# jtdingx/quadrupedal_loco

Measured on AMD Instinct MI355X. Metric: MPC QP solves/sec (Go1 SRBD N=10, 12 forces); p99 solve us, higher is better.
Workload: dtype f32

## Files before the change

### quadrupedal_loco_amd/csrc/qloco_srbd_lit.hip

```cpp
#include <math.h>
#include <stddef.h>

#include <type_traits>

#include "qloco_srbd_core.hpp"
#include "qloco_srbd_model.hpp"
#include "qloco_srbd_place.hpp"

namespace qloco {

constexpr int kLitWpe = 4;
constexpr int kLit2Wpe = 2;

template <int W>
struct LitLds {
  static constexpr int NS = W == 1 ? kLitN : kLitN2;
  static constexpr int NT = NS;
  float Bb[6][12];
  float Te[6][6];
  float q2[16], r2[12], x0[16];
  float ctf[4 * NT];
  float pad0[W == 1 ? 0 : 24];
  f4v bc[W][W][16];
  float av[W][2][64];
  float wv[W][64];
  float zh[W][2][64];
  float dr[W][2][64];
  float qvl[W][2][64];
  f4v arz[W][2][64];
  union alignas(16) {
    struct {
      f2v beps[12][12];
      float dcol[12 * NT];
      float err[12 * NT];
      float Wc[12 * NT];
    };
    struct {
      float w0i[W][3][2][64];
      f2v gtab[NT][NT][3];
    };
  };
  f2v k0k2[NT][NT];
  struct {
    float rho, cs, cinv, qn0, qn1, alpha, oma, sigma, dtm;
    float zlo;
    float sxy[2][2];
    int iter, status, rho_updates, ctm, interval;
  } sc[W];
  float piv[W == 1 ? 0 : 2];
  float red[W == 1 ? 0 : 2][16];
};
static_assert(sizeof(LitLds<1>) <= 10240, "literal kernel: four workgroups per SIMD need <= 160 KB / 16 of LDS");
static_assert(sizeof(LitLds<2>) <= 40960, "two-wave literal kernel: four workgroups per CU need <= 40 KB");
static_assert(offsetof(LitLds<1>, dcol) % 16 == 0 && offsetof(LitLds<2>, dcol) % 16 == 0,
              "dcol is read as f4v (ds_read_b128 needs 16-byte alignment)");
static_assert(offsetof(LitLds<1>, Bb) % 16 == 0 && offsetof(LitLds<1>, bc) % 16 == 0 && offsetof(LitLds<1>, arz) % 16 == 0 &&
                  offsetof(LitLds<2>, Bb) % 16 == 0 && offsetof(LitLds<2>, bc) % 16 == 0 && offsetof(LitLds<2>, arz) % 16 == 0,
              "Bb rows, bc and arz are read as f4v");
static_assert((offsetof(LitLds<1>, w0i) - offsetof(LitLds<1>, bc)) % 256 == 0 &&
                  (offsetof(LitLds<2>, w0i) - offsetof(LitLds<2>, bc)) % 256 == 0 && offsetof(LitLds<1>, Bb) == 0,
              "the ADMM loop's two-address reads reach its per-lane arrays from one lane register");

__device__ __forceinline__ void lsync() {
  __builtin_amdgcn_fence(__ATOMIC_RELEASE, "wavefront");
  __builtin_amdgcn_wave_barrier();
  __builtin_amdgcn_fence(__ATOMIC_ACQUIRE, "wavefront");
}
template <int W>
__device__ __forceinline__ void bsync() {
  if constexpr (W == 1)
    lsync();
  else
    __syncthreads();
}

template <int W, int K>
__device__ __forceinline__ void bcombine_max(LitLds<W> &S, float (&v)[K], int wv) {
  if constexpr (W == 2) {
    static_assert(K <= 16, "red holds 16 partials per wave");
    if (__builtin_amdgcn_mbcnt_hi(~0u, __builtin_amdgcn_mbcnt_lo(~0u, 0u)) == 0) {
#pragma unroll
      for (int k = 0; k < K; ++k) S.red[wv][k] = v[k];
    }
    bsync<W>();
#pragma unroll
    for (int k = 0; k < K; ++k) v[k] = fmaxf(S.red[0][k], S.red[1][k]);
    bsync<W>();
  }
}
template <int W>
__device__ __forceinline__ float bsum(LitLds<W> &S, float v, int wv) {
  if constexpr (W == 2) {
    if (__builtin_amdgcn_mbcnt_hi(~0u, __builtin_amdgcn_mbcnt_lo(~0u, 0u)) == 0) S.red[wv][0] = v;
    bsync<W>();
    v = S.red[0][0] + S.red[1][0];
    bsync<W>();
  }
  return v;
}
template <int W>
__device__ __forceinline__ float bmax1(LitLds<W> &S, float v, int wv) {
  float t[1] = {v};
  bcombine_max<W, 1>(S, t, wv);
  return t[0];
}

struct Triple {
  float v0, v1, v2;
};
__device__ __forceinline__ Triple triple(float v, int comp) {
  const float n1 = lane_next(v), n2 = lane_next(n1);
  const float p1 = lane_prev(v), p2 = lane_prev(p1);
  Triple t;
  t.v0 = comp == 0 ? v : (comp == 1 ? p1 : p2);
  t.v1 = comp == 0 ? n1 : (comp == 1 ? v : p1);
  t.v2 = comp == 0 ? n2 : (comp == 1 ? n1 : v);
  return t;
}

struct Shift5 {
  float cm2, cm1, c0, cp1, cp2;
};
__device__ __forceinline__ Shift5 shift5(float a0, float a1, float a2, int comp) {
  Shift5 c;
  c.c0 = comp == 0 ? a0 : (comp == 1 ? a1 : a2);
  c.cm1 = comp == 1 ? a0 : (comp == 2 ? a1 : 0.0f);
  c.cm2 = comp == 2 ? a0 : 0.0f;
  c.cp1 = comp == 0 ? a1 : (comp == 1 ? a2 : 0.0f);
  c.cp2 = comp == 0 ? a2 : 0.0f;
  return c;
}
__device__ __forceinline__ float tdot(float v, const Shift5 &c) {
  float a, t, u;
  asm("s_nop 1\n\t"
      "v_mov_b32_dpp %1, %3 wave_shr:1 row_mask:0xf bank_mask:0xf bound_ctrl:0\n\t"
      "v_mov_b32_dpp %2, %3 wave_shl:1 row_mask:0xf bank_mask:0xf bound_ctrl:0\n\t"
      "v_mul_f32 %0, %3, %4\n\t"
      "v_fmac_f32_dpp %0, %3, %5 wave_shr:1 row_mask:0xf bank_mask:0xf bound_ctrl:0\n\t"
      "v_fmac_f32_dpp %0, %3, %7 wave_shl:1 row_mask:0xf bank_mask:0xf bound_ctrl:0\n\t"
      "v_fmac_f32_dpp %0, %1, %6 wave_shr:1 row_mask:0xf bank_mask:0xf bound_ctrl:0\n\t"
      "v_fmac_f32_dpp %0, %2, %8 wave_shl:1 row_mask:0xf bank_mask:0xf bound_ctrl:0"
      : "=&v"(a), "=&v"(t), "=&v"(u)
      : "v"(v), "v"(c.c0), "v"(c.cm1), "v"(c.cm2), "v"(c.cp1), "v"(c.cp2));
  return a;
}

__device__ __forceinline__ void tdot2(float v0, const Shift5 &c, float v1, const Shift5 &d, float &a0, float &a1) {
  float t0, t1, u0, u1;
  asm("s_nop 1\n\t"
      "v_mov_b32_dpp %2, %6 wave_shr:1 row_mask:0xf bank_mask:0xf bound_ctrl:0\n\t"
      "v_mov_b32_dpp %3, %7 wave_shr:1 row_mask:0xf bank_mask:0xf bound_ctrl:0\n\t"
      "v_mov_b32_dpp %4, %6 wave_shl:1 row_mask:0xf bank_mask:0xf bound_ctrl:0\n\t"
      "v_mov_b32_dpp %5, %7 wave_shl:1 row_mask:0xf bank_mask:0xf bound_ctrl:0\n\t"
      "v_mul_f32 %0, %6, %8\n\t"
      "v_mul_f32 %1, %7, %13\n\t"
      "v_fmac_f32_dpp %0, %6, %9 wave_shr:1 row_mask:0xf bank_mask:0xf bound_ctrl:0\n\t"
      "v_fmac_f32_dpp %1, %7, %14 wave_shr:1 row_mask:0xf bank_mask:0xf bound_ctrl:0\n\t"
      "v_fmac_f32_dpp %0, %6, %11 wave_shl:1 row_mask:0xf bank_mask:0xf bound_ctrl:0\n\t"
      "v_fmac_f32_dpp %1, %7, %16 wave_shl:1 row_mask:0xf bank_mask:0xf bound_ctrl:0\n\t"
      "v_fmac_f32_dpp %0, %2, %10 wave_shr:1 row_mask:0xf bank_mask:0xf bound_ctrl:0\n\t"
      "v_fmac_f32_dpp %1, %3, %15 wave_shr:1 row_mask:0xf bank_mask:0xf bound_ctrl:0\n\t"
      "v_fmac_f32_dpp %0, %4, %12 wave_shl:1 row_mask:0xf bank_mask:0xf bound_ctrl:0\n\t"
      "v_fmac_f32_dpp %1, %5, %17 wave_shl:1 row_mask:0xf bank_mask:0xf bound_ctrl:0"
      : "=&v"(a0), "=&v"(a1), "=&v"(t0), "=&v"(t1), "=&v"(u0), "=&v"(u1)
      : "v"(v0), "v"(v1), "v"(c.c0), "v"(c.cm1), "v"(c.cm2), "v"(c.cp1), "v"(c.cp2),
        "v"(d.c0), "v"(d.cm1), "v"(d.cm2), "v"(d.cp1), "v"(d.cp2));
}

__device__ __forceinline__ void lit_invert(LitLds<1> &S, int lane, int ncol, Row<1> &K) {
  int nc = __builtin_amdgcn_readfirstlane(ncol);
  {
    const float v = K.k[0];
    const float p = __builtin_bit_cast(float, __builtin_amdgcn_readlane(__builtin_bit_cast(int, v), 0));
    reinterpret_cast<float *>(&S.bc[0][0][0])[lane] = lane == 0 ? p + 1.0f : v;
  }
  ColLoop<0, 60>::run([&](auto kc) {
    constexpr int k = decltype(kc)::value;
    asm volatile("" : "+s"(nc));
    if (k >= nc) return;
    const bool is_k = __builtin_amdgcn_inverse_ballot_w64(1ull << k);
    lsync();
    const f4v r0 = S.bc[0][0][lane & 15];
    const float v = K.k[k];
    const float p = __builtin_bit_cast(float, __builtin_amdgcn_readlane(__builtin_bit_cast(int, v), k));
    const float pinv = __builtin_amdgcn_rcpf(p);
    const float ng = is_k ? pinv - 1.0f : -v * pinv;
    if constexpr (k + 1 < 60) {
      const bool is_k1 = __builtin_amdgcn_inverse_ballot_w64(1ull << (k + 1));
      const bool upto_k = __builtin_amdgcn_inverse_ballot_w64((2ull << k) - 1ull);
      const float la = fmaf(dpp_col<k + 1>(r0), ng, K.k[k + 1]);
      const float p1 = __builtin_bit_cast(float, __builtin_amdgcn_readlane(__builtin_bit_cast(int, la), k + 1));
      reinterpret_cast<float *>(&S.bc[0][0][0])[lane] = is_k1 ? p1 + 1.0f : (upto_k ? -la : la);
    }
    QL_DPP_GJ60_P1(K.k, 0, r0, ng);
    if (p > kGjExactPivot) K.k[k] = is_k ? pinv : ng;
  });
  lsync();
}

template <int HF, int KL>
__device__ __forceinline__ void lit2_pivot(LitLds<2> &S, int wv, int nc, Row<2> &K) {
  const int tt = fresh_lane();
  if constexpr (KL >= 1) {
    if (KL == nc) {
      constexpr int k1 = 60 * HF + KL - 1;
      const float v = K.k[k1];
      const bool own1 = wv == HF && tt == KL - 1;
      const bool before = HF == 0 && wv == 1;
      reinterpret_cast<float *>(&S.bc[k1 & 1][wv][0])[tt] = own1 ? v + 1.0f : (before ? -v : v);
      if (own1) S.piv[k1 & 1] = v;
    }
  }
  if constexpr (KL < 60) {
    constexpr int k = 60 * HF + KL;
    constexpr int pb = k & 1;
    if (KL >= nc) return;
    bsync<2>();
    const f4v r0 = S.bc[pb][0][tt & 15];
    const f4v r1 = S.bc[pb][1][tt & 15];
    const float p = S.piv[pb];
    const float v = K.k[k];
    const float pinv = __builtin_amdgcn_rcpf(p);
    const bool own = wv == HF && tt == KL;
    const float ng = own ? pinv - 1.0f : -v * pinv;
    if constexpr (KL >= 1) {
      const float la = fmaf(dpp_col<KL - 1>(HF ? r1 : r0), ng, K.k[k - 1]);
      const bool own1 = wv == HF && tt == KL - 1;
      const bool before = HF ? (wv == 1 && tt >= KL) : (wv == 1 || tt >= KL);
      reinterpret_cast<float *>(&S.bc[pb ^ 1][wv][0])[tt] = own1 ? la + 1.0f : (before ? -la : la);
      if (own1) S.piv[pb ^ 1] = la;
    }
    QL_DPP_GJ60(K.k, 0, r0, ng);
    QL_DPP_GJ60(K.k, 60, r1, ng);
    if (p > kGjExactPivot) K.k[k] = own ? pinv : ng;
  }
}

__device__ __forceinline__ void lit_invert2(LitLds<2> &S, int wv, int nc0, int nc1, Row<2> &K) {
  nc0 = __builtin_amdgcn_readfirstlane(nc0);
  nc1 = __builtin_amdgcn_readfirstlane(nc1);
  ColLoop<0, 61>::run([&](auto kc) {
    asm volatile("" : "+s"(nc1));
    lit2_pivot<1, 60 - decltype(kc)::value>(S, wv, nc1, K);
  });
  ColLoop<0, 61>::run([&](auto kc) {
    asm volatile("" : "+s"(nc0));
    lit2_pivot<0, 60 - decltype(kc)::value>(S, wv, nc0, K);
  });
  bsync<2>();
}

#define QL_LIT_LANE_INDICES(LX)                                                                    \
  const int LX = fresh_lane();                                                                     \
  const int jr = LX < 60 ? LX / 6 : kLitN - 1, sr = LX < 60 ? LX - 6 * (LX / 6) : 0;               \
  const int jc = W == 1 ? jr : 10 * wv + jr;                                                       \
  const bool wvalid = LX < nw;                                                                     \
  const int step[2] = {LX < 60 && LX < nvl ? so + LX / 12 : so, LX < 60 && 60 + LX < nvl ? so + (60 + LX) / 12 : so}; \
  const int stepl[2] = {step[0] - so, step[1] - so};                                               \
  const int leg[2] = {LX < 60 && LX < nvl ? (LX % 12) / 3 : 0, LX < 60 && 60 + LX < nvl ? ((60 + LX) % 12) / 3 : 0}; \
  const int comp = LX % 3;                                                                         \
  const bool xy = comp < 2;                                                                        \
  const bool valid[2] = {LX < 60 && LX < nvl, LX < 60 && 60 + LX < nvl};                           \
  (void)jr; (void)sr; (void)jc; (void)wvalid; (void)stepl; (void)step; (void)leg; (void)comp; (void)xy; (void)valid

template <int W, bool WS, bool MR>
__device__ __forceinline__ void srbd_lit_one(const SrbdArgs &a, LitLds<W> &S, const int64_t b) {
  constexpr int NS = LitLds<W>::NS, NT = LitLds<W>::NT;
  const int lane = W == 1 ? (int)threadIdx.x : (int)(threadIdx.x & 63);
  const int tid = threadIdx.x;
  const int wv = W == 1 ? 0 : __builtin_amdgcn_readfirstlane((int)(threadIdx.x >> 6));
  const int N = a.N;
  const float Nf = (float)N;
  const float dt = a.dt;
  SrbdBodyAt<MR> body{a};
  auto load_body = [&] {
    if constexpr (MR) {
      int64_t bb = b;
      asm volatile("" : "+s"(bb));
      body.row = srbd_body(a, bb);
    }
  };
  if constexpr (MR) {
    body.row = srbd_body(a, b);
    if (srbd_body_bad(body.row)) {
      srbd_refuse<64 * W>(a, b, W == 1 ? fresh_lane() : opaque_tid(), QLOCO_ERR_ARG);
      return;
    }
  }
  const float dtm = dt / body.mass(), dt2m = dt * dt / body.mass();
  const int H = W == 1 ? N : (N + 1) / 2;
  const int so = W == 1 ? 0 : wv * H;
  const int Nw = W == 1 ? N : (wv ? N - H : H);
  const int nvar = 12 * N, nvl = 12 * Nw, nw = 6 * Nw;

  if (tid < 13) S.x0[tid] = a.x0[b * 13 + tid];
  if (tid == 0) {
#pragma unroll
    for (int k = 0; k < 13; ++k) S.q2[k] = a.q2[k];
#pragma unroll
    for (int k = 0; k < 12; ++k) S.r2[k] = a.r2[k];
  }
  {
    const int nct = a.contacts_per_step ? 4 * N : 4;
    if (tid < 4 * N) S.ctf[tid] = a.contacts[b * nct + (a.contacts_per_step ? tid : (tid & 3))] ? 1.0f : 0.0f;
  }
  for (int idx = tid; idx < NT * NT; idx += 64 * W) {
    const int sr = idx / NT, sc = idx - NT * sr;
    float K0 = 0.0f, K2 = 0.0f;
    if constexpr (W == 1) {
      if (sr < N && sc < N) k0k2((float)sr, (float)sc, Nf, K0, K2);
    } else {
      const int gr = sr % 10 < (sr >= 10 ? N - H : H) ? (sr >= 10 ? H : 0) + sr % 10 : -1;
      const int gc = sc % 10 < (sc >= 10 ? N - H : H) ? (sc >= 10 ? H : 0) + sc % 10 : -1;
      if (gr >= 0 && gc >= 0) k0k2((float)gr, (float)gc, Nf, K0, K2);
    }
    S.k0k2[sr][sc] = (f2v){K0, K2};
  }
  if constexpr (W == 2) {
    for (int idx = tid; idx < 12 * NT; idx += 64 * W) S.dcol[idx] = 0.0f;
  }
  bsync<W>();

  const float yaw = S.x0[2];
  float sy, cy;
  sincosf(yaw, &sy, &cy);
  const float R00 = cy, R01 = sy, R10 = -sy, R11 = cy;
  if constexpr (W == 1) {
    if (a.lit_tables && tid == 0) {
      const float sq = a.lit_sq;
      S.sc[0].sxy[0][0] = sq * cy;
      S.sc[0].sxy[0][1] = -(sq * sy);
      S.sc[0].sxy[1][0] = sq * sy;
      S.sc[0].sxy[1][1] = sq * cy;
    }
  }
  float Ii[3][3];
  srbd_inertia_inv(cy, sy, body.inertia(), Ii);
  const int comp = lane % 3;
  const bool xy = comp < 2;
  bool valid[2];
  int step[2], leg[2], cst[2];
  f4v lo[2], hi[2];
#pragma unroll
  for (int h = 0; h < 2; ++h) {
    const int v = 60 * h + lane;
    valid[h] = lane < 60 && v < nvl;
    step[h] = valid[h] ? so + v / 12 : 0;
    cst[h] = W == 1 ? step[h] : (valid[h] ? 10 * wv + v / 12 : 0);
    leg[h] = valid[h] ? (v % 12) / 3 : 0;
    float ba[3];
    srbd_bd_column(Ii, srbd_foot(a.feet, b, N, 0, step[h], leg[h]), comp, dt, R00, R01, R10, R11,
                   step[h], valid[h], ba, lo[h], hi[h]);
    if (h == 0 && tid < 12) {
      S.Bb[0][lane] = ba[0];
      S.Bb[1][lane] = ba[1];
      S.Bb[2][lane] = ba[2];
      S.Bb[3][lane] = comp == 0 ? dtm : 0.0f;
      S.Bb[4][lane] = comp == 1 ? dtm : 0.0f;
      S.Bb[5][lane] = comp == 2 ? dtm : 0.0f;
    }
  }
  if (tid < 36) {
    const int r = lane / 6, c = lane - 6 * (lane / 6);
    const float Rm[3][3] = {{R00, R01, 0.f}, {R10, R11, 0.f}, {0.f, 0.f, 1.f}};
    float v = 0.0f;
    if (r < 3 && c < 3)
      v = dt * dt * (Rm[0][r] * S.q2[0] * Rm[0][c] + Rm[1][r] * S.q2[1] * Rm[1][c] + Rm[2][r] * S.q2[2] * Rm[2][c]);
    else if (r >= 3 && c == r)
      v = dt * dt * S.q2[r];
    S.Te[r][c] = v;
  }
  float r2v[2];
#pragma unroll
  for (int h = 0; h < 2; ++h) r2v[h] = valid[h] ? S.r2[3 * leg[h] + comp] : 0.0f;

  for (int idx = tid; idx < 12 * N; idx += 64 * W) {
    const int i = idx / 12, s = idx - 12 * i;
    const float xf = srbd_free_state<12>(S.x0, s, i, dt, R00, R01, R10, R11);
    S.err[idx] = S.q2[s] * (xf - a.xref[b * 13 * N + 13 * i + s]);
  }
  bsync<W>();
  if (tid < 12) {
    const int r = lane;
    const bool brow = r >= 6;
    float s0 = 0.0f, s1 = 0.0f;
#pragma unroll
    for (int j = NS - 1; j >= 0; --j) {
      if (j < N) {
        s1 += s0;
        s0 += S.err[12 * j + r];
        S.Wc[12 * j + r] = brow ? s0 : s1;
      }
    }
  }
  bsync<W>();
  float qv[2], qsv[2];
#pragma unroll
  for (int h = 0; h < 2; ++h) {
    float g = 0.0f;
    if (valid[h]) {
      const float *w = S.Wc + 12 * step[h];
      g = lo[h].x * w[6] + lo[h].y * w[7] + lo[h].z * w[8];
      g += lo[h].w * w[0] + hi[h].x * w[1] + hi[h].y * w[2];
      g += dtm * w[9 + comp] + dt2m * w[3 + comp];
    }
    qv[h] = g;
    qsv[h] = g;
  }
  const int NP = 100 * N;
  float *prec = (WS && a.warm_start == 2) ? a.warm + b * (int64_t)(NP + 4) : nullptr;
  bool p_init = false;
  if (prec) p_init = prec[NP + 1] > 0.5f;
  const bool p_same = p_init;
  if (p_same) {
#pragma unroll
    for (int h = 0; h < 2; ++h)
      if (valid[h]) qsv[h] = prec[84 * N + 12 * step[h] + 3 * leg[h] + comp];
  }
  if (prec) {
#pragma unroll
    for (int h = 0; h < 2; ++h)
      if (valid[h]) prec[84 * N + 12 * step[h] + 3 * leg[h] + comp] = qv[h];
  }

  float ra0[2], ra1[2], rz0[2], rz1[2], rl0[2], ru0[2];
  load_body();
#pragma unroll
  for (int h = 0; h < 2; ++h) {
    ra0[h] = valid[h] ? 1.0f : 0.0f;
    ra1[h] = (valid[h] && xy) ? 1.0f : 0.0f;
    rz0[h] = (valid[h] && xy) ? body.mu() : 0.0f;
    rz1[h] = (valid[h] && xy) ? -body.mu() : 0.0f;
    const float cflag = valid[h] ? S.ctf[4 * step[h] + leg[h]] : 0.0f;
    rl0[h] = !valid[h] ? 0.0f : (xy ? 0.0f : body.fz_min() * cflag);
    ru0[h] = !valid[h] ? 0.0f : (xy ? INFINITY : body.fz_max() * cflag);
  }

  float rE0[2] = {1.0f, 1.0f}, rE1[2] = {1.0f, 1.0f}, Dr[2] = {1.0f, 1.0f}, cs = 1.0f;
  {
    bsync<W>();
    for (int e = tid; e < 144; e += 64 * W) {
      const int w = e / 12, wp = e - 12 * (e / 12);
      float bb = 0.0f, ee = 0.0f;
#pragma unroll
      for (int s = 0; s < 6; ++s) {
        bb = fmaf(S.q2[6 + s] * S.Bb[s][w], S.Bb[s][wp], bb);
        float tw = 0.0f;
#pragma unroll
        for (int t = 0; t < 6; ++t) tw = fmaf(S.Te[s][t], S.Bb[t][wp], tw);
        ee = fmaf(S.Bb[s][w], tw, ee);
      }
      S.beps[w][wp] = (f2v){bb, ee};
    }
    bsync<W>();
    float pdiag[2];
#pragma unroll
    for (int h = 0; h < 2; ++h) {
      const int wl = valid[h] ? (60 * h + lane) % 12 : 0;
      const f2v kk = S.k0k2[cst[h]][cst[h]];
      const f2v be = S.beps[wl][wl];
      pdiag[h] = valid[h] ? fmaf(kk.y, be.y, kk.x * be.x) + r2v[h] : 0.0f;
    }
    f2v be2[6], ep2[6];
    {
      const int wl = lane < 60 ? lane % 12 : 0;
#pragma unroll
      for (int p = 0; p < 6; ++p) {
        const f4v q = *reinterpret_cast<const f4v *>(&S.beps[wl][2 * p]);
        be2[p] = (f2v){q.x, q.z};
        ep2[p] = (f2v){q.y, q.w};
      }
    }
    auto row_norms = [&](bool scaled, float (&m)[2]) {
#pragma unroll
      for (int p = 0; p < 6; ++p) asm volatile("" : "+v"(be2[p]), "+v"(ep2[p]));
      float ma[2] = {0.0f, 0.0f}, mb[2] = {0.0f, 0.0f};
      const f4v one4 = (f4v)(1.0f);
      f2v k0 = S.k0k2[cst[0]][0], k1 = S.k0k2[cst[1]][0];
      f4v da = scaled ? reinterpret_cast<const f4v *>(&S.dcol[0])[0] : one4,
          db = scaled ? reinterpret_cast<const f4v *>(&S.dcol[0])[1] : one4,
          dd = scaled ? reinterpret_cast<const f4v *>(&S.dcol[0])[2] : one4;
#pragma unroll
      for (int kc = 0; kc < NS; ++kc) {
        const int kn = kc + 1 < NS ? kc + 1 : kc;
        asm volatile("" ::: "memory");
        const f2v k0n = S.k0k2[cst[0]][kn], k1n = S.k0k2[cst[1]][kn];
        const f4v *dcn = reinterpret_cast<const f4v *>(&S.dcol[12 * kn]);
        const f4v dan = scaled ? dcn[0] : one4, dbn = scaled ? dcn[1] : one4, ddn = scaled ? dcn[2] : one4;
        __builtin_amdgcn_sched_barrier(0);
        const f2v dv[6] = {{da.x, da.y}, {da.z, da.w}, {db.x, db.y}, {db.z, db.w}, {dd.x, dd.y}, {dd.z, dd.w}};
#pragma unroll
        for (int g = 0; g < 3; ++g) {
          f2v t[4];
#pragma unroll
          for (int c = 0; c < 4; ++c) t[c] = (f2v)((c >> 1) ? k1.x : k0.x) * be2[2 * g + (c & 1)];
          __builtin_amdgcn_sched_barrier(0);
#pragma unroll
          for (int c = 0; c < 4; ++c)
            t[c] = __builtin_elementwise_fma((f2v)((c >> 1) ? k1.y : k0.y), ep2[2 * g + (c & 1)], t[c]);
          __builtin_amdgcn_sched_barrier(0);
// ... 207 lines not shown
      const float Dinvl = __builtin_amdgcn_rcpf(Drl);
      const f4v arz = S.arz[wv][h][lxr];
      const f2v Einv = {valid[h] ? Drl * __builtin_amdgcn_rcpf(arz.x) : 1.0f,
                        (valid[h] && xy) ? Drl * __builtin_amdgcn_rcpf(arz.y) : 1.0f};
      const f2v ra = {arz.x, arz.y}, rz = {arz.z, arz.w};
      const float n1 = lane_next(x[h]), n2 = lane_next(n1);
      const float xz = comp == 0 ? n2 : (comp == 1 ? n1 : x[h]);
      const f2v ay = ra * y[h], az = rz * y[h];
      const float ay_z = az.x + az.y;
      const float p1 = lane_prev(ay_z), p2 = lane_prev(p1);
      const float aty = valid[h] ? ((ay.x + ay.y) + (comp == 2 ? (p1 + p2) : 0.0f)) : 0.0f;
      const float rd = valid[h] ? (S.qvl[wv][h][lxr] + px[h] + aty) : 0.0f;
      const f2v ax = ra * x[h] + rz * xz;
      const f2v rp = ax - z[h];
      const f2v erp = Einv * rp, ez = Einv * z[h], eax = Einv * ax;
      o[0] = fmaxf(o[0], fmaxf(fabsf(erp.x), fabsf(erp.y)));
      o[1] = fmaxf(o[1], fmaxf(fabsf(ez.x), fabsf(ez.y)));
      o[2] = fmaxf(o[2], fmaxf(fabsf(eax.x), fabsf(eax.y)));
      o[3] = fmaxf(o[3], fabsf(Dinvl * rd));
      o[4] = fmaxf(o[4], fabsf(Dinvl * aty));
      o[5] = fmaxf(o[5], fabsf(Dinvl * px[h]));
      if (want_r) {
        r[0] = fmaxf(r[0], fmaxf(fabsf(rp.x), fabsf(rp.y)));
        r[1] = fmaxf(r[1], fmaxf(fabsf(z[h].x), fabsf(z[h].y)));
        r[2] = fmaxf(r[2], fmaxf(fabsf(ax.x), fabsf(ax.y)));
        r[3] = fmaxf(r[3], fabsf(rd));
        r[4] = fmaxf(r[4], fabsf(aty));
        r[5] = fmaxf(r[5], fabsf(px[h]));
      }
    }
    wmax_nonneg6(o);
    if (want_r) wmax_nonneg6(r);
    if constexpr (W == 2) {
      float v[12];
#pragma unroll
      for (int k = 0; k < 6; ++k) v[k] = o[k], v[6 + k] = want_r ? r[k] : 0.0f;
      bcombine_max<W, 12>(S, v, wv);
#pragma unroll
      for (int k = 0; k < 6; ++k) o[k] = v[k], r[k] = v[6 + k];
    }
  };

  if (WS) {
    QL_LIT_LANE_INDICES(lxs);
#pragma unroll
    for (int h = 0; h < 2; ++h) {
      const int vidx = 12 * step[h] + 3 * leg[h] + comp, rbase = 20 * step[h] + 5 * leg[h] + 2 * comp;
      if (p_same) {
        x[h] = valid[h] ? prec[vidx] : 0.0f;
        z[h].x = valid[h] ? prec[12 * N + rbase] : 0.0f;
        z[h].y = (valid[h] && xy) ? prec[12 * N + rbase + 1] : 0.0f;
        y[h].x = valid[h] ? prec[32 * N + rbase] : 0.0f;
        y[h].y = (valid[h] && xy) ? prec[32 * N + rbase + 1] : 0.0f;
      } else if (a.warm_start == 1) {
        const float *wx = a.warm + b * (32 * N);
        const float *wy = wx + 12 * N;
        x[h] = valid[h] ? wx[vidx] / S.dr[wv][h][lxs] : 0.0f;
        const f2v e = row_e(h);
        const float csl = uf(S.sc[wv].cs);
        y[h].x = valid[h] ? wy[rbase] / e.x * csl : 0.0f;
        y[h].y = (valid[h] && xy) ? wy[rbase + 1] / e.y * csl : 0.0f;
        const float n1 = lane_next(x[h]), n2 = lane_next(n1);
        const float xz = comp == 0 ? n2 : (comp == 1 ? n1 : x[h]);
        const f4v arz = S.arz[wv][h][lxs];
        z[h] = (f2v){arz.x, arz.y} * x[h] + (f2v){arz.z, arz.w} * xz;
      }
    }
  }
  float gmx = 0.0f;
  bool host_tables = false;
  if constexpr (W == 1) host_tables = a.lit_tables != 0;
  if (host_tables) {
    if constexpr (W == 1) {
      static_assert(sizeof(S.gtab) == sizeof(a.lit_gtab) && offsetof(LitLds<1>, gtab) % 16 == 0 &&
                        offsetof(SrbdArgs, lit_gtab) % 16 == 0,
                    "the host tables are copied as f4v into gtab");
      constexpr int NV = (int)(sizeof(a.lit_gtab) / (sizeof(float) * 4));
      const int fl = fresh_lane();
      typedef const f4v __attribute__((address_space(4))) *KernargF4;
      typedef const char __attribute__((address_space(4))) *KernargBytes;
      const KernargBytes args = (KernargBytes)__builtin_amdgcn_kernarg_segment_ptr();
      const KernargF4 src = (KernargF4)(args + offsetof(SrbdArgs, lit_gtab));
      f4v *dst = reinterpret_cast<f4v *>(&S.gtab[0][0][0]);
#pragma unroll
      for (int i = 0; i < (NV + 63) / 64; ++i)
        if (64 * i + fl < NV) dst[64 * i + fl] = src[64 * i + fl];
      gmx = sgpr_f(a.lit_gmx);
      bsync<W>();
    }
  } else {
    double row[NS];
    const int r = tid;
    const bool live = r < 6 * N;
    const int ax = live ? r / N : 0, ri = live ? r - N * (r / N) : 0;
    double sxy[2][2], sn2 = 1.0;
    {
      const double dt2 = (double)dt * (double)dt;
      double lam[2];
      {
        const double qx = (double)S.q2[6], qy = (double)S.q2[7];
        const double yw = (double)S.x0[2], cw = cos(yw), sw = sin(yw);
        const double Rm[2][2] = {{cw, sw}, {-sw, cw}};
        double T[2][2];
#pragma unroll
        for (int i = 0; i < 2; ++i)
#pragma unroll
          for (int j = 0; j < 2; ++j)
            T[i][j] = Rm[0][i] * (double)S.q2[0] * Rm[0][j] + Rm[1][i] * (double)S.q2[1] * Rm[1][j];
        const double ix = 1.0 / sqrt(qx), iy = 1.0 / sqrt(qy);
        const double c00 = T[0][0] * ix * ix, c01 = T[0][1] * ix * iy, c11 = T[1][1] * iy * iy;
        double t = 0.0;
        if (c01 != 0.0) {
          const double tau = (c11 - c00) / (2.0 * c01);
          t = tau == 0.0 ? 1.0 : (tau > 0.0 ? 1.0 : -1.0) / (fabs(tau) + sqrt(1.0 + tau * tau));
        }
        const double cs = 1.0 / sqrt(1.0 + t * t), sn = t * cs;
        lam[0] = c00 - t * c01;
        lam[1] = c11 + t * c01;
        sxy[0][0] = ix * cs;
        sxy[0][1] = ix * sn;
        sxy[1][0] = -iy * sn;
        sxy[1][1] = iy * cs;
        if (ax < 2) sn2 = sxy[0][ax] * sxy[0][ax] + sxy[1][ax] * sxy[1][ax];
      }
      const double al = ax < 2 ? 1.0 : (ax == 2 ? (double)S.q2[8] : (double)S.q2[9 + ax - 3]);
      const double be = ax < 2 ? dt2 * lam[ax] : dt2 * (double)S.q2[ax];
#pragma unroll
      for (int k = 0; k < NS; ++k) {
        const int M = ri > k ? ri : k;
        const double T0 = (double)(N - M), ia = (double)(M - ri), ib = (double)(M - k);
        const double S1 = 0.5 * T0 * (T0 - 1.0), S2 = (T0 - 1.0) * T0 * (2.0 * T0 - 1.0) / 6.0;
        const double K2 = S2 + (ia + ib) * S1 + ia * ib * T0;
        row[k] = (live && k < N) ? fma(al, T0, be * K2) : (k == ri ? 1.0 : 0.0);
      }
    }
    double *xch = reinterpret_cast<double *>(&S.gtab[0][0][0]);
    static_assert(sizeof(S.gtab) >= 2 * 6 * NS * sizeof(double), "pivot-row exchange fits the table area");
#pragma unroll
    for (int k = 0; k < NS; ++k) {
      if (k >= N) continue;
      double *buf = xch + (k & 1) * (6 * NS);
      if (live && ri == k) {
#pragma unroll
        for (int c = 0; c < NS; ++c) buf[ax * NS + c] = row[c];
      }
      bsync<W>();
      const double *pr = buf + ax * NS;
      const double pinv = 1.0 / pr[k];
      const double fk = row[k] * pinv;
#pragma unroll
      for (int c = 0; c < NS; ++c) {
        if (c == k) continue;
        const double pc = pr[c];
        row[c] = ri == k ? pc * pinv : fma(-fk, pc, row[c]);
      }
      row[k] = ri == k ? pinv : -fk;
    }
    bsync<W>();
    for (int idx = tid; idx < NT * NT * 3; idx += 64 * W) (&S.gtab[0][0][0])[idx] = (f2v)(0.0f);
    bsync<W>();
    float dmax = 0.0f;
    if (live) {
      const int csi = W == 1 ? ri : (ri < H ? ri : 10 + ri - H);
      float *dst = reinterpret_cast<float *>(&S.gtab[csi][0][0]);
#pragma unroll
      for (int k = 0; k < NS; ++k) {
        if (k < N) {
          const int csk = W == 1 ? k : (k < H ? k : 10 + k - H);
          dst[csk * 6 + ax] = (float)row[k];
        }
        dmax = k == ri ? (float)(sn2 * row[k]) : dmax;
      }
    }
    if (tid == 0) {
#pragma unroll
      for (int i = 0; i < 2; ++i)
#pragma unroll
        for (int j = 0; j < 2; ++j) S.sc[wv].sxy[i][j] = (float)sxy[i][j];
    }
    if constexpr (W == 2) {
      if (tid == 64) {
#pragma unroll
        for (int i = 0; i < 2; ++i)
#pragma unroll
          for (int j = 0; j < 2; ++j) S.sc[1].sxy[i][j] = (float)sxy[i][j];
      }
    }
    gmx = sgpr_f(bmax1<W>(S, wmax_nonneg(dmax), wv));
    bsync<W>();
  }
  for (;;) {
    {
      int ln = fresh_lane();
      asm volatile("" : "+v"(ln));
      const float rho = uf(S.sc[wv].rho), cinv = uf(S.sc[wv].cinv), sigma = uf(S.sc[wv].sigma);
      QL_LIT_LANE_INDICES(lxf);
      auto w0_inv_row = [&](int h, float &i0, float &i1, float &i2) {
        const float dinv_h = valid[h] ? 1.0f / S.dr[wv][h][lxf] : 0.0f, csw = uf(S.sc[wv].cs);
        const f4v arz = S.arz[wv][h][lxf];
        const float rv0 = eq0[h] ? 1e3f * rho : rho, rv1 = rho;
        const float d_own = rv0 * arz.x * arz.x + rv1 * arz.y * arz.y;
        const float d_oz = rv0 * arz.x * arz.z + rv1 * arz.y * arz.w;
        const float d_zz = rv0 * arz.z * arz.z + rv1 * arz.w * arz.w;
        const float oz1 = lane_prev(d_oz), oz2 = lane_prev(oz1);
        const float zz1 = lane_prev(d_zz), zz2 = lane_prev(zz1);
        float m0, m1, m2;
        if (comp == 0) {
          m0 = d_own + sigma; m1 = 0.0f; m2 = d_oz;
        } else if (comp == 1) {
          m0 = 0.0f; m1 = d_own + sigma; m2 = d_oz;
        } else {
          m0 = oz2; m1 = oz1; m2 = d_own + zz1 + zz2 + sigma;
        }
        const Triple dd = triple(dinv_h, comp);
        float w0 = dinv_h * m0 * dd.v0, w1 = dinv_h * m1 * dd.v1, w2 = dinv_h * m2 * dd.v2;
        const float cr = csw * (valid[h] ? S.r2[3 * leg[h] + comp] : 0.0f);
        w0 += comp == 0 ? cr : 0.0f;
        w1 += comp == 1 ? cr : 0.0f;
        w2 += comp == 2 ? cr : 0.0f;
        if (!valid[h]) { w0 = comp == 0 ? 1.0f : 0.0f; w1 = comp == 1 ? 1.0f : 0.0f; w2 = comp == 2 ? 1.0f : 0.0f; }
        const Triple c0 = triple(w0, comp), c1 = triple(w1, comp), c2 = triple(w2, comp);
        const float a00 = c0.v0, a01 = c1.v0, a02 = c2.v0;
        const float a10 = c0.v1, a11 = c1.v1, a12 = c2.v1;
        const float a20 = c0.v2, a21 = c1.v2, a22 = c2.v2;
        const float k00 = a11 * a22 - a12 * a21, k01 = a02 * a21 - a01 * a22, k02 = a01 * a12 - a02 * a11;
        const float k10 = a12 * a20 - a10 * a22, k11 = a00 * a22 - a02 * a20, k12 = a02 * a10 - a00 * a12;
        const float k20 = a10 * a21 - a11 * a20, k21 = a01 * a20 - a00 * a21, k22 = a00 * a11 - a01 * a10;
        const float idet = 1.0f / (a00 * k00 + a01 * k10 + a02 * k20);
        i0 = (comp == 0 ? k00 : (comp == 1 ? k10 : k20)) * idet;
        i1 = (comp == 0 ? k01 : (comp == 1 ? k11 : k21)) * idet;
        i2 = (comp == 0 ? k02 : (comp == 1 ? k12 : k22)) * idet;
      };
#pragma unroll
      for (int h = 0; h < 2; ++h) {
        float i0, i1, i2;
        w0_inv_row(h, i0, i1, i2);
        S.w0i[wv][0][h][lxf] = i0;
        S.w0i[wv][1][h][lxf] = i1;
        S.w0i[wv][2][h][lxf] = i2;
      }
      lsync();
      float Urow[6];
      {
        float yv[12];
        const int hh = jr >= 5 ? 1 : 0, base = 12 * (jr - 5 * hh);
#pragma unroll
        for (int g = 0; g < 4; ++g) {
          const int v0 = base + 3 * g;
          const f4v r0 = {S.w0i[wv][0][hh][v0], S.w0i[wv][1][hh][v0], S.w0i[wv][2][hh][v0], 0.0f},
                    r1 = {S.w0i[wv][0][hh][v0 + 1], S.w0i[wv][1][hh][v0 + 1], S.w0i[wv][2][hh][v0 + 1], 0.0f},
                    r2 = {S.w0i[wv][0][hh][v0 + 2], S.w0i[wv][1][hh][v0 + 2], S.w0i[wv][2][hh][v0 + 2], 0.0f};
          const float b0 = S.Bb[sr][3 * g], b1 = S.Bb[sr][3 * g + 1], b2 = S.Bb[sr][3 * g + 2];
          yv[3 * g + 0] = b0 * r0.x + b1 * r1.x + b2 * r2.x;
          yv[3 * g + 1] = b0 * r0.y + b1 * r1.y + b2 * r2.y;
          yv[3 * g + 2] = b0 * r0.z + b1 * r1.z + b2 * r2.z;
        }
#pragma unroll
        for (int t = 0; t < 6; ++t) {
          float acc = 0.0f;
#pragma unroll
          for (int w = 0; w < 12; ++w) acc = fmaf(yv[w], S.Bb[t][w], acc);
          Urow[t] = wvalid ? acc : (t == sr ? 1.0f : 0.0f);
        }
      }
      float sM;
      {
        float uii = 0.0f;
#pragma unroll
        for (int t = 0; t < 6; ++t) uii = t == sr ? Urow[t] : uii;
        sM = sgpr_f(1.0f / fmaf(gmx, cinv, bmax1<W>(S, wmax_nonneg(wvalid ? uii : 0.0f), wv)));
        const float s00 = uf(S.sc[wv].sxy[0][0]), s01 = uf(S.sc[wv].sxy[0][1]), s10 = uf(S.sc[wv].sxy[1][0]),
                    s11 = uf(S.sc[wv].sxy[1][1]);
        const float r0 = !wvalid ? 0.0f : (sr == 0 ? s00 : (sr == 1 ? s10 : 0.0f)),
                    r1 = !wvalid ? 0.0f : (sr == 0 ? s01 : (sr == 1 ? s11 : 0.0f));
        const float c00 = r0 * s00, c01 = r0 * s10, c10 = r1 * s01, c11 = r1 * s11;
        const float m2 = (wvalid && sr == 2) ? 1.0f : 0.0f, m3 = (wvalid && sr == 3) ? 1.0f : 0.0f,
                    m4 = (wvalid && sr == 4) ? 1.0f : 0.0f, m5 = (wvalid && sr == 5) ? 1.0f : 0.0f;
        const float scale = sM * cinv;
        const float unit = (!wvalid && ln < 60) ? 1.0f : 0.0f;
        float own_add[6];
#pragma unroll
        for (int t = 0; t < 6; ++t) own_add[t] = fmaf(scale, t == sr ? unit : 0.0f, sM * Urow[t]);
#pragma unroll
        for (int wp = 0; wp < W; ++wp) {
#pragma unroll
          for (int k = 0; k < kLitN; ++k) {
            const f2v e0 = S.gtab[jc][10 * wp + k][0], e1 = S.gtab[jc][10 * wp + k][1],
                      e2 = S.gtab[jc][10 * wp + k][2];
            const float gv[6] = {fmaf(c00, e0.x, c10 * e0.y), fmaf(c01, e0.x, c11 * e0.y), m2 * e1.x,
                                 m3 * e1.y, m4 * e2.x, m5 * e2.y};
            const bool blk = wp == wv && k == jr;
#pragma unroll
            for (int t = 0; t < 6; ++t) {
              const int c = 60 * wp + 6 * k + t;
              T.k[c] = fmaf(scale, gv[t], blk ? own_add[t] : 0.0f);
              asm volatile("" : "+v"(T.k[c]));
            }
          }
        }
#pragma unroll
        for (int c = 60 * W; c < 64 * W; ++c) T.k[c] = 0.0f;
      }
      if constexpr (W == 1)
        lit_invert(S, lxf, nw, T);
      else
        lit_invert2(S, wv, 6 * H, 6 * (N - H), T);
#pragma unroll
      for (int c = 0; c < 60 * W; ++c) T.k[c] *= sM;
#pragma unroll
      for (int h = 0; h < 2; ++h) {
        const float wx = S.w0i[wv][0][h][lxf], wy = S.w0i[wv][1][h][lxf], wz = S.w0i[wv][2][h][lxf];
        W1[h] = shift5(valid[h] ? wx : 0.0f, valid[h] ? wy : 0.0f, valid[h] ? wz : 0.0f, comp);
      }
    }
    bool refactor = false;

    for (;;) {
      int iter = ui(S.sc[wv].iter);
      const int ctm = ui(S.sc[wv].ctm), interval = ui(S.sc[wv].interval);
      if (iter < a.max_iter) {
        int next = a.max_iter;
        if (ctm) next = min(next, (iter / ctm + 1) * ctm);
        if (interval) next = min(next, (iter / interval + 1) * interval);
        const float rho = uf(S.sc[wv].rho);
        const float rho_s = rho;
        const float rvb_s = sgpr_f(1.0f / rho);
        const float zlo = uf(S.sc[wv].zlo);
        QL_LIT_LANE_INDICES(lxi);
        const float alpha = uf(S.sc[wv].alpha), oma = uf(S.sc[wv].oma), sigma = uf(S.sc[wv].sigma),
                    dtm = uf(S.sc[wv].dtm);
        float qvr[2], Dinv[2];
#pragma unroll
        for (int h = 0; h < 2; ++h) {
          qvr[h] = S.qvl[wv][h][lxi];
          Dinv[h] = valid[h] ? 1.0f / S.dr[wv][h][lxi] : 0.0f;
          S.w0i[wv][0][h][lxi] = Dinv[h];
          S.w0i[wv][1][h][lxi] = xy ? 0.0f : zlo * S.zh[wv][h][lxi];
        }
        float rva0[2], rvia[2];
#pragma unroll
        for (int h = 0; h < 2; ++h) {
          rva0[h] = eq0[h] ? 1e3f * rho_s : rho_s;
          rvia[h] = eq0[h] ? 1e-3f * rvb_s : rvb_s;
          asm volatile("" : "+v"(rva0[h]), "+v"(rvia[h]));
        }
        iter = __builtin_amdgcn_readfirstlane(iter);
        next = __builtin_amdgcn_readfirstlane(next);
        __builtin_amdgcn_sched_barrier(0);
        f4v arzc[2] = {S.arz[wv][0][lxi], S.arz[wv][1][lxi]};
        const uint64_t xym = __builtin_amdgcn_ballot_w64(xy);
        for (; iter < next; ++iter) {
          asm volatile("" ::: "memory");
          const int par = W == 1 ? 0 : (iter & 1);
          const float rva[2][2] = {{rva0[0], rho_s}, {rva0[1], rho_s}};
          const float rvb = rvb_s;
          float av[2];
          float tz[2], rhs[2];
#pragma unroll
          for (int h = 0; h < 2; ++h) {
            const f2v ra = {arzc[h].x, arzc[h].y}, rz = {arzc[h].z, arzc[h].w};
            const f2v rv = {rva[h][0], rva[h][1]};
            const f2v w = __builtin_elementwise_fma(rv, z[h], -y[h]);
            const f2v aw = ra * w, zw = rz * w;
            tz[h] = zw.x + zw.y;
            rhs[h] = fmaf(sigma, x[h], (aw.x + aw.y) - qvr[h]);
          }
          const f4v *br = reinterpret_cast<const f4v *>(S.Bb[sr]);
          const f4v b0 = br[0], b1 = br[1], b2 = br[2];
          __builtin_amdgcn_sched_barrier(0);
          {
            float m2, u0, u1, t0, t1;
            asm volatile("v_cndmask_b32_e64 %0, 1.0, 0, %1" : "=v"(m2) : "s"(xym));
            asm("s_nop 1\n\t"
                "v_add_f32_dpp %2, %8, %8 wave_shr:1 row_mask:0xf bank_mask:0xf bound_ctrl:0\n\t"
                "v_add_f32_dpp %3, %9, %9 wave_shr:1 row_mask:0xf bank_mask:0xf bound_ctrl:0\n\t"
                "s_nop 0\n\t"
                "v_fmac_f32_dpp %4, %2, %10 wave_shr:1 row_mask:0xf bank_mask:0xf bound_ctrl:0\n\t"
                "v_fmac_f32_dpp %5, %3, %10 wave_shr:1 row_mask:0xf bank_mask:0xf bound_ctrl:0\n\t"
                "v_mul_f32 %6, %11, %4\n\t"
                "v_mul_f32 %7, %12, %5\n\t"
                "s_nop 0\n\t"
                "v_mov_b32_dpp %2, %6 wave_shr:1 row_mask:0xf bank_mask:0xf bound_ctrl:0\n\t"
                "v_mov_b32_dpp %3, %7 wave_shr:1 row_mask:0xf bank_mask:0xf bound_ctrl:0\n\t"
                "v_mov_b32_dpp %4, %6 wave_shl:1 row_mask:0xf bank_mask:0xf bound_ctrl:0\n\t"
                "v_mov_b32_dpp %5, %7 wave_shl:1 row_mask:0xf bank_mask:0xf bound_ctrl:0\n\t"
                "v_mul_f32 %0, %6, %13\n\t"
                "v_mul_f32 %1, %7, %18\n\t"
                "v_fmac_f32_dpp %0, %6, %14 wave_shr:1 row_mask:0xf bank_mask:0xf bound_ctrl:0\n\t"
                "v_fmac_f32_dpp %1, %7, %19 wave_shr:1 row_mask:0xf bank_mask:0xf bound_ctrl:0\n\t"
                "v_fmac_f32_dpp %0, %6, %16 wave_shl:1 row_mask:0xf bank_mask:0xf bound_ctrl:0\n\t"
                "v_fmac_f32_dpp %1, %7, %21 wave_shl:1 row_mask:0xf bank_mask:0xf bound_ctrl:0\n\t"
                "v_fmac_f32_dpp %0, %2, %15 wave_shr:1 row_mask:0xf bank_mask:0xf bound_ctrl:0\n\t"
                "v_fmac_f32_dpp %1, %3, %20 wave_shr:1 row_mask:0xf bank_mask:0xf bound_ctrl:0\n\t"
                "v_fmac_f32_dpp %0, %4, %17 wave_shl:1 row_mask:0xf bank_mask:0xf bound_ctrl:0\n\t"
                "v_fmac_f32_dpp %1, %5, %22 wave_shl:1 row_mask:0xf bank_mask:0xf bound_ctrl:0"
                : "=&v"(av[0]), "=&v"(av[1]), "=&v"(u0), "=&v"(u1), "+v"(rhs[0]), "+v"(rhs[1]), "=&v"(t0), "=&v"(t1)
                : "v"(tz[0]), "v"(tz[1]), "v"(m2), "v"(Dinv[0]), "v"(Dinv[1]),
                  "v"(W1[0].c0), "v"(W1[0].cm1), "v"(W1[0].cm2), "v"(W1[0].cp1), "v"(W1[0].cp2),
                  "v"(W1[1].c0), "v"(W1[1].cm1), "v"(W1[1].cm2), "v"(W1[1].cp1), "v"(W1[1].cp2));
          }
          S.av[wv][0][lxi] = av[0];
          S.av[wv][1][lxi] = av[1];
          lsync();
          float wr = 0.0f;
          {
            const int hh = jr >= 5 ? 1 : 0, base = 12 * (jr - 5 * hh);
            const f4v *src = reinterpret_cast<const f4v *>(&S.av[wv][hh][base]);
            const f4v u0 = src[0], u1 = src[1];
            f4v u2;
            if constexpr (W == 2) u2 = src[2];
            __builtin_amdgcn_sched_barrier(0);
            float w0 = 0.0f, w1 = 0.0f;
            w0 = fmaf(b0.x, u0.x, w0);
            w1 = fmaf(b0.y, u0.y, w1);
            w0 = fmaf(b0.z, u0.z, w0);
            w1 = fmaf(b0.w, u0.w, w1);
            if constexpr (W == 1) {
              __builtin_amdgcn_sched_barrier(0);
              u2 = src[2];
              __builtin_amdgcn_sched_barrier(0);
            }
            w0 = fmaf(b1.x, u1.x, w0);
            w1 = fmaf(b1.y, u1.y, w1);
            w0 = fmaf(b1.z, u1.z, w0);
            w1 = fmaf(b1.w, u1.w, w1);
            w0 = fmaf(b2.x, u2.x, w0);
            w1 = fmaf(b2.y, u2.y, w1);
            w0 = fmaf(b2.z, u2.z, w0);
            w1 = fmaf(b2.w, u2.w, w1);
            wr = w0 + w1;
          }
          reinterpret_cast<float *>(&S.bc[par][wv][0])[lxi] = wr;
          bsync<W>();
          float sv;
          float bw0, bw1, bw2, zhi[2], zlw[2], avr[2];
          {
            const f4v r0 = S.bc[par][0][lxi & 15];
            f4v r1;
            if constexpr (W == 2) r1 = S.bc[par][1][lxi & 15];
            bw0 = S.Bb[0][lxi % 12], bw1 = S.Bb[1][lxi % 12], bw2 = S.Bb[2][lxi % 12];
#pragma unroll
            for (int h = 0; h < 2; ++h) {
              avr[h] = S.av[wv][h][lxi];
              Dinv[h] = S.w0i[wv][0][h][lxi];
            }
            __builtin_amdgcn_sched_barrier(0);
            float acc0, acc1;
            QL_DPP_MATVEC60_2(acc0, acc1, r0, T.k, 0);
            if constexpr (W == 2) {
              float acc2, acc3;
              QL_DPP_MATVEC60_2(acc2, acc3, r1, T.k, 60);
              sv = (acc0 + acc1) + (acc2 + acc3);
            } else {
              sv = acc0 + acc1;
            }
          }
          S.wv[wv][lxi] = sv;
          lsync();
          f2v s01[2];
          float s2[2], sf[2];
          {
            const float *gs = &S.wv[wv][6 * stepl[0]], *gc = gs + 3 + comp;
#pragma unroll
            for (int h = 0; h < 2; ++h) sf[h] = gc[30 * h];
            __builtin_amdgcn_sched_barrier(0);
#pragma unroll
            for (int h = 0; h < 2; ++h) s2[h] = gs[30 * h + 2];
            __builtin_amdgcn_sched_barrier(0);
#pragma unroll
            for (int h = 0; h < 2; ++h) s01[h] = *reinterpret_cast<const f2v *>(gs + 30 * h);
            __builtin_amdgcn_sched_barrier(0);
          }
          float tv[2], td[2];
#pragma unroll
          for (int h = 0; h < 2; ++h)
            tv[h] = fmaf(bw0, s01[h].x, fmaf(bw1, s01[h].y, fmaf(bw2, s2[h], dtm * sf[h])));
          asm volatile("" : "+v"(tv[0]), "+v"(tv[1]));
          arzc[0] = S.arz[wv][0][lxi];
          arzc[1] = S.arz[wv][1][lxi];
          __builtin_amdgcn_sched_barrier(0);
          tdot2(tv[0], W1[0], tv[1], W1[1], td[0], td[1]);
#pragma unroll
          for (int h = 0; h < 2; ++h) {
            zhi[h] = S.zh[wv][h][lxi];
            zlw[h] = S.w0i[wv][1][h][lxi];
            qvr[h] = S.qvl[wv][h][lxi];
          }
          float xt[2], xtz[2];
          f2v zt[2], zr[2], vv[2], zn[2];
#pragma unroll
          for (int h = 0; h < 2; ++h) xt[h] = Dinv[h] * (avr[h] - td[h]);
#pragma unroll
          for (int h = 0; h < 2; ++h) {
            const float n1 = lane_next(xt[h]), n2 = lane_next(n1);
            xtz[h] = comp == 0 ? n2 : n1;
            x[h] = fmaf(alpha, xt[h], oma * x[h]);
          }
          asm volatile("" : "+v"(arzc[0]), "+v"(arzc[1]));
#pragma unroll
          for (int h = 0; h < 2; ++h) {
            const f2v ra = {arzc[h].x, arzc[h].y}, rz = {arzc[h].z, arzc[h].w};
            zt[h] = __builtin_elementwise_fma(rz, (f2v)(xtz[h]), ra * xt[h]);
          }
#pragma unroll
          for (int h = 0; h < 2; ++h) zr[h] = __builtin_elementwise_fma((f2v)(alpha), zt[h], oma * z[h]);
#pragma unroll
          for (int h = 0; h < 2; ++h) {
            const f2v rvi2 = {rvia[h], rvb};
            vv[h] = __builtin_elementwise_fma(y[h], rvi2, zr[h]);
          }
#pragma unroll
          for (int h = 0; h < 2; ++h)
            zn[h] = {__builtin_amdgcn_fmed3f(vv[h].x, zlw[h], zhi[h]), __builtin_amdgcn_fmed3f(vv[h].y, -INFINITY, 0.0f)};
#pragma unroll
          for (int h = 0; h < 2; ++h) {
            const f2v rv = {rva[h][0], rva[h][1]};
            y[h] = __builtin_elementwise_fma(rv, zr[h] - zn[h], y[h]);
            z[h] = zn[h];
          }
        }
      }
      iter = ui(iter);
      S.sc[wv].iter = iter;
      const bool fin = iter >= a.max_iter;
      const bool can_check = ctm && iter > 0 && (iter % ctm == 0);
      const bool do_rho = interval && iter > 0 && (iter % interval == 0);
      if (!(can_check || do_rho || fin)) continue;
      float o[6], r[6];
      residuals(o, r, do_rho);
      const float cinv = uf(S.sc[wv].cinv), qn0 = uf(S.sc[wv].qn0);
      const float pri_res = o[0], dua_res = cinv * o[3];
      if (can_check) {
        const float eps_p = a.eps_abs + a.eps_rel * fmaxf(o[1], o[2]);
        const float eps_d = a.eps_abs + a.eps_rel * cinv * fmaxf(fmaxf(qn0, o[4]), o[5]);
        if (pri_res < eps_p && dua_res < eps_d) {
          S.sc[wv].status = QLOCO_OK;
          break;
        }
      }
      if (do_rho) {
        const float pn = r[0] / (fmaxf(r[1], r[2]) + 1e-30f);
        const float dn = r[3] / (fmaxf(fmaxf(uf(S.sc[wv].qn1), r[4]), r[5]) + 1e-30f);
        const float rho = uf(S.sc[wv].rho);
        float rho_new = rho * sqrtf(pn / (dn + 1e-30f));
        rho_new = fminf(fmaxf(rho_new, 1e-6f), 1e6f);
        if (rho_new > rho * a.rho_tol || rho_new < rho / a.rho_tol) {
          const int nup = ui(S.sc[wv].rho_updates) + 1;
          S.sc[wv].rho = sgpr_f(rho_new);
          S.sc[wv].rho_updates = nup;
          if (!fin) {
            refactor = true;
            break;
          }
        }
      }
      if (fin) {
        float e_abs = a.eps_abs, e_rel = a.eps_rel;
        asm volatile("" : "+v"(e_abs), "+v"(e_rel));
        const float ep = 10.f * e_abs + 10.f * e_rel * fmaxf(o[1], o[2]);
        const float ed = 10.f * e_abs + 10.f * e_rel * cinv * fmaxf(fmaxf(qn0, o[4]), o[5]);
        S.sc[wv].status = __builtin_amdgcn_readfirstlane((pri_res < ep && dua_res < ed) ? QLOCO_SOLVED_INACCURATE
                                                                                          : QLOCO_MAX_ITER);
        break;
      }
    }
    if (!refactor) break;
  }

  const int lane_o = fresh_lane();
  const int tid_o = W == 1 ? lane_o : (int)threadIdx.x;
  float xu[2];
#pragma unroll
  for (int h = 0; h < 2; ++h) xu[h] = valid[h] ? x[h] * S.dr[wv][h][lane_o] : 0.0f;
  float px[2];
  p_times_x(px);
  const float cinv = uf(S.sc[wv].cinv);
  int status = ui(S.sc[wv].status);
  float ob = 0.0f;
#pragma unroll
  for (int h = 0; h < 2; ++h) ob += valid[h] ? cinv * (0.5f * x[h] * px[h] + S.qvl[wv][h][lane_o] * x[h]) : 0.0f;
  const float objp = bsum<W>(S, wsum(ob), wv);
  const bool bad = !isfinite(objp);
  if (bad) status = QLOCO_NAN;
  if (a.u) {
    float *uo = a.u + b * 12 * N + 12 * so;
#pragma unroll
    for (int h = 0; h < 2; ++h)
      if (valid[h]) uo[60 * h + lane_o] = bad ? NAN : xu[h];
  }
  {
    const float n1 = lane_next(xu[0]), n2 = lane_next(n1);
    const float p1 = lane_prev(xu[0]), p2 = lane_prev(p1);
    const float f0 = comp == 0 ? xu[0] : (comp == 1 ? p1 : p2);
    const float f1 = comp == 0 ? n1 : (comp == 1 ? xu[0] : p1);
    const float f2 = comp == 0 ? n2 : (comp == 1 ? n1 : xu[0]);
    if (tid_o < 12) {
      float o = xu[0];
      if (a.output_frame == 1) {
        const float yw = S.x0[2], cw = cosf(yw), sw = sinf(yw);
        o = comp == 0 ? (cw * f0 - sw * f1) : (comp == 1 ? (sw * f0 + cw * f1) : f2);
      }
      a.u0[b * 12 + lane_o] = bad ? NAN : o;
    }
  }
  if (prec) {
    QL_LIT_LANE_INDICES(lxo);
    for (int k = tid_o; k < NP + 4; k += 64 * W)
// ... 149 lines not shown
```

Before: 12.13 million.

## Perform Gauss-Jordan inversion rank-1 updates with MFMA 32x32x1 outer products

Replaces the per-column LDS broadcast plus DPP fused-multiply-add update in the single-wave Gauss-Jordan inverse with two MFMA 32x32x1 rank-1 updates per pivot. The matrix is remapped into the MFMA accumulator layout using permlane32 swaps before and after the loop, which removes the LDS round trip and barriers on every pivot. In exchange it adds layout-conversion overhead and serial MFMA latency on each pivot step, and it depends on the accumulator layout being mapped correctly.

```diff
diff --git a/quadrupedal_loco_amd/csrc/qloco_srbd_lit.hip b/quadrupedal_loco_amd/csrc/qloco_srbd_lit.hip
--- a/quadrupedal_loco_amd/csrc/qloco_srbd_lit.hip
+++ b/quadrupedal_loco_amd/csrc/qloco_srbd_lit.hip
@@ -167,35 +167,84 @@
         "v"(d.c0), "v"(d.cm1), "v"(d.cm2), "v"(d.cp1), "v"(d.cp2));
 }
 
-__device__ __forceinline__ void lit_invert(LitLds<1> &S, int lane, int ncol, Row<1> &K) {
+typedef float f32x32 __attribute__((ext_vector_type(32)));
+__device__ __forceinline__ void lit_swap32(float &a, float &b) {
+  const auto r = __builtin_amdgcn_permlane32_swap(__builtin_bit_cast(unsigned, a), __builtin_bit_cast(unsigned, b), false, false);
+  const unsigned r0 = r[0], r1 = r[1];
+  a = __builtin_bit_cast(float, r0);
+  b = __builtin_bit_cast(float, r1);
+}
+constexpr int lit_gj_j0(int q) { return (q & 3) + 8 * (q >> 2); }
+
+template <int k>
+__device__ __forceinline__ void lit_pivot(f32x32 &D1, f32x32 &D2) {
+  constexpr int jb = k >> 5, kk = k & 31, h = (kk >> 2) & 1, q = (kk & 3) + 4 * (kk >> 3);
+  static_assert(lit_gj_j0(q) + 4 * h == kk, "column k: register q of the blocks (jb, .), lane half h");
+  constexpr int x = jb == 0 ? q : 16 + q;
+  const bool is_k = __builtin_amdgcn_inverse_ballot_w64(1ull << k);
+  const bool before_k = __builtin_amdgcn_inverse_ballot_w64((1ull << k) - 1ull);
+  const bool lo = __builtin_amdgcn_inverse_ballot_w64(0xffffffffull);
+  float X = jb == 0 ? D1[x] : D2[x], Y = jb == 0 ? D2[x] : D1[x];
+  lit_swap32(X, Y);
+  const float v = h == 0 ? X : Y;
+  const float p = __builtin_bit_cast(float, __builtin_amdgcn_readlane(__builtin_bit_cast(int, v), k));
+  const float pinv = __builtin_amdgcn_rcpf(p);
+  const float ng = is_k ? pinv - 1.0f : -v * pinv;
+  const float c = is_k ? p + 1.0f : (before_k ? -v : v);
+  float nl = ng, nh = ng;
+  lit_swap32(nl, nh);
+  const float ngs = lo ? nh : nl;
+  D1 = __builtin_amdgcn_mfma_f32_32x32x1f32(c, ng, D1, 0, 0, 0);
+  D2 = __builtin_amdgcn_mfma_f32_32x32x1f32(c, ngs, D2, 0, 0, 0);
+  if (p > kGjExactPivot) {
+    const bool is_ks = __builtin_amdgcn_inverse_ballot_w64(1ull << (k ^ 32));
+    const bool half_h = h == 0 ? lo : !lo;
+    const float e = is_k ? pinv : ng, es = is_ks ? pinv : ngs;
+    const float e0 = h == 0 ? e : es, e1 = h == 0 ? es : e;
+    if constexpr (jb == 0) {
+      D1[x] = half_h ? e0 : D1[x];
+      D2[x] = half_h ? e1 : D2[x];
+    } else {
+      D2[x] = half_h ? e0 : D2[x];
+      D1[x] = half_h ? e1 : D1[x];
+    }
+  }
+}
+
+__device__ __forceinline__ void lit_invert(int ncol, Row<1> &K) {
   int nc = __builtin_amdgcn_readfirstlane(ncol);
-  {
-    const float v = K.k[0];
-    const float p = __builtin_bit_cast(float, __builtin_amdgcn_readlane(__builtin_bit_cast(int, v), 0));
-    reinterpret_cast<float *>(&S.bc[0][0][0])[lane] = lane == 0 ? p + 1.0f : v;
+  f32x32 D1, D2;
+#pragma unroll
+  for (int jb = 0; jb < 2; ++jb) {
+#pragma unroll
+    for (int q = 0; q < 16; ++q) {
+      float a = K.k[32 * jb + lit_gj_j0(q)], b = K.k[32 * jb + lit_gj_j0(q) + 4];
+      lit_swap32(a, b);
+      if (jb == 0) {
+        D1[q] = a;
+        D2[q] = b;
+      } else {
+        D2[16 + q] = a;
+        D1[16 + q] = b;
+      }
+    }
   }
   ColLoop<0, 60>::run([&](auto kc) {
     constexpr int k = decltype(kc)::value;
     asm volatile("" : "+s"(nc));
     if (k >= nc) return;
-    const bool is_k = __builtin_amdgcn_inverse_ballot_w64(1ull << k);
-    lsync();
-    const f4v r0 = S.bc[0][0][lane & 15];
-    const float v = K.k[k];
-    const float p = __builtin_bit_cast(float, __builtin_amdgcn_readlane(__builtin_bit_cast(int, v), k));
-    const float pinv = __builtin_amdgcn_rcpf(p);
-    const float ng = is_k ? pinv - 1.0f : -v * pinv;
-    if constexpr (k + 1 < 60) {
-      const bool is_k1 = __builtin_amdgcn_inverse_ballot_w64(1ull << (k + 1));
-      const bool upto_k = __builtin_amdgcn_inverse_ballot_w64((2ull << k) - 1ull);
-      const float la = fmaf(dpp_col<k + 1>(r0), ng, K.k[k + 1]);
-      const float p1 = __builtin_bit_cast(float, __builtin_amdgcn_readlane(__builtin_bit_cast(int, la), k + 1));
-      reinterpret_cast<float *>(&S.bc[0][0][0])[lane] = is_k1 ? p1 + 1.0f : (upto_k ? -la : la);
-    }
-    QL_DPP_GJ60_P1(K.k, 0, r0, ng);
-    if (p > kGjExactPivot) K.k[k] = is_k ? pinv : ng;
+    lit_pivot<k>(D1, D2);
   });
-  lsync();
+#pragma unroll
+  for (int jb = 0; jb < 2; ++jb) {
+#pragma unroll
+    for (int q = 0; q < 16; ++q) {
+      float a = jb == 0 ? D1[q] : D2[16 + q], b = jb == 0 ? D2[q] : D1[16 + q];
+      lit_swap32(a, b);
+      K.k[32 * jb + lit_gj_j0(q)] = a;
+      K.k[32 * jb + lit_gj_j0(q) + 4] = b;
+    }
+  }
 }
 
 template <int HF, int KL>
@@ -1009,7 +1058,7 @@
         for (int c = 60 * W; c < 64 * W; ++c) T.k[c] = 0.0f;
       }
       if constexpr (W == 1)
-        lit_invert(S, lxf, nw, T);
+        lit_invert(nw, T);
       else
         lit_invert2(S, wv, 6 * H, 6 * (N - H), T);
 #pragma unroll
```

New measurement: 12.68 million, median of 6. 1.05x the previous value.
